# JoshuaQSH/FALCON-TTDforGNNs

Measured on NVIDIA B200. Metric: TT-EmbeddingBag rows/s fwd+bwd+SGD, higher is better.
Workload: dtype f32

## Files before the change

falcon-ttdforgnns_b200/csrc/common.cuh:

```cuda
#pragma once

#include <cuda_runtime.h>
#include <stdint.h>
#include <stdio.h>
#include <string.h>

#include "../../include/ttg_b200.h"

#if defined(__CUDA_ARCH__) && (__CUDA_ARCH__ < 1000)
#error "ttg_b200 is written for sm_100a (B200) only"
#endif

namespace ttg {

constexpr int kWarp = 32;
constexpr int kNumSMs = 148;

void set_error(const char* fmt, ...);
void count_launch(int n = 1);

#define TTG_CHECK_ARG(cond, ...)  \
  do {                            \
    if (!(cond)) {                \
      ttg::set_error(__VA_ARGS__); \
// ... 151 lines not shown
struct MmaPlan {
  const uint32_t* skeys;
  const int32_t* srow;
  const int32_t* cnt;
  const int32_t* base;
  float* Ttab;
  float* S;
  float* d0parts;
  uint32_t first_key;
  int32_t spare_sms;
};
bool mma_supported(const TTDev& tt);
bool mma_fwd_supported(const TTDev& tt);
int mma_table(const TTDev& tt, const MmaPlan& pl, bool tf32, bool chained, cudaStream_t stream);
int mma_forward(const TTDev& tt, int64_t nnz, uint32_t total_rows, const MmaPlan& pl, float* output,
                bool tf32, cudaStream_t stream);
int mma_backward(const TTDev& tt, int64_t nnz, uint32_t total_rows, const MmaPlan& pl,
                 const float* d_output, float* const* dcore, int32_t optim, float lr, float eps,
                 float* const* state, bool tf32, cudaStream_t stream);

int mma_cores_finalize(const TTDev& tt, const MmaPlan& pl, float* const* dcore, int32_t optim, float lr,
                       float eps, float* const* state, bool tf32, cudaStream_t stream);

struct RPlan {
  const uint32_t* skeys;
  const int32_t* srow;
  const int32_t* cnt;
  const int32_t* base;
  float* tab;
  float* S1;
  float* d0parts;
  float* d2parts;
};
bool r_supported(const TTDev& tt);
// ... 16 lines not shown
```

falcon-ttdforgnns_b200/csrc/tt_mma.cu:

```cuda
#include <stdlib.h>

#include <type_traits>

#include "common.cuh"

namespace ttg {

namespace {

constexpr int kThreads = 512;
constexpr int kWarps = kThreads / 32;
constexpr int kCoreThreads = 256;
constexpr int cores_warps(int c) { return c <= 80 ? 16 : 8; }
constexpr int kCoreWarps = kCoreThreads / 32;
constexpr uint32_t kInvalid = 0xffffffffu;
constexpr size_t kSmemMax = 227 * 1024;

template <int TERMS>
struct Frag {
  uint32_t hi, lo;
  __device__ __forceinline__ void set(float x) {
    if (TERMS == 3) {
      hi = (__float_as_uint(x) + 0x1000u) & 0xffffe000u;
      lo = __float_as_uint(x - __uint_as_float(hi));
// ... 85 lines not shown
          smem_u32(sdst)),
      "l"(gsrc), "r"(bytes), "r"(smem_u32(bar))
      : "memory");
}
__device__ __forceinline__ void mbar_wait(uint64_t* bar, uint32_t parity) {
  asm volatile(
      "{\n"
      ".reg .pred p;\n"
      "WAIT_%=:\n"
      "mbarrier.try_wait.parity.shared::cta.b64 p, [%0], %1;\n"
      "@p bra DONE_%=;\n"
      "bra WAIT_%=;\n"
      "DONE_%=:\n"
      "}\n" ::"r"(smem_u32(bar)),
      "r"(parity)
      : "memory");
}

constexpr int kStageU = 6;
template <int NT, typename F>
__device__ __forceinline__ void stage_core2(const float* __restrict__ core2, int nelem, F&& put) {
  const int n4 = nelem / 4;
  for (int base4 = 0; base4 < n4; base4 += NT * kStageU) {
    float4 v[kStageU];
#pragma unroll
    for (int u = 0; u < kStageU; ++u) {
      const int i4 = base4 + u * NT + (int)threadIdx.x;
      v[u] = (i4 < n4) ? ldg4(core2 + 4 * i4) : make_float4(0.f, 0.f, 0.f, 0.f);
    }
#pragma unroll
// ... 112 lines not shown
          b[1].set_split(bh.y, 0.f);
        }
        mma_terms<TERMS>(acc, a[ks], b);
      }
      if (d0) *reinterpret_cast<float2*>(d0 + 8 * nt) = make_float2(acc[0], acc[1]);
      if (d1) *reinterpret_cast<float2*>(d1 + 8 * nt) = make_float2(acc[2], acc[3]);
    }
  }
}

constexpr int tile_rows(int q2) { return 16 / q2; }
constexpr int fwd_rb(int q2) { return (16 / tile_rows(q2)) * tile_rows(q2); }
constexpr int bwd_rb(int q2) { return (q2 <= 5 ? 3 : 4) * tile_rows(q2); }
constexpr int kC2Stride = 20;

struct PairSlot {
  int row;
  int j2;
};
template <int Q2>
__device__ __forceinline__ PairSlot pair_slot(int p) {
  PairSlot s;
  s.row = p / Q2;
  s.j2 = p - s.row * Q2;
  if (p >= tile_rows(Q2) * Q2) {
    s.row = 99;
    s.j2 = 0;
  }
  return s;
}

template <int Q0, int Q1, int Q2, int R2, int TERMS, bool C2S>
__global__ void __launch_bounds__(kThreads, 1)
mma_fwd_kernel(TTDev tt, int64_t nnz, uint32_t total_rows, const uint32_t* __restrict__ skeys,
               const int32_t* __restrict__ srow, const float* __restrict__ Ttab,
               float* __restrict__ output, int rows_per_warp, int npairs_c2, int dbg,
               uint32_t first_key) {
  constexpr int A = Q0 * Q1;
  constexpr int D = A * Q2;
  constexpr int NTL = (A + 7) / 8;
  constexpr int KS = R2 / 8;
  constexpr int TR = tile_rows(Q2);
  constexpr int RB = fwd_rb(Q2);
  constexpr int CS = kC2Stride;
  static_assert(R2 % 8 == 0 && (!C2S || R2 == 16), "shared-memory core2 layout is written for r2 = 16");
  static_assert(D % 4 == 0 && A % 2 == 0 && 2 * RB <= 32, "layout");
  extern __shared__ __align__(128) float smem[];
  float* c2hi = smem;
  float* c2lo = smem + (size_t)npairs_c2 * CS;
  float* stage_all = smem + (C2S ? (size_t)npairs_c2 * CS * (TERMS == 3 ? 2 : 1) : 0);

  const int lane = threadIdx.x & 31, wib = threadIdx.x >> 5;
  const int gid = lane >> 2, tid = lane & 3;
  pdl_trigger();
  if (C2S) {
    stage_core2<kThreads>(tt.core[2], npairs_c2 * 16, [&](int e, float v) {
      const int i2row = e / (16 * Q2), rem = e % (16 * Q2);
      const int k2 = rem / Q2, j2 = rem % Q2;
      const int dst = (i2row * Q2 + j2) * CS + k2;
      if (TERMS == 3) {
        const float hi = tf32_hi(v);
        c2hi[dst] = hi;
        c2lo[dst] = v - hi;
      } else {
        c2hi[dst] = __uint_as_float(__float_as_uint(v) + 0x1000u);
      }
    });
    __syncthreads();
  }
  pdl_wait();

  const uint32_t p2 = tt.p[2];
  const uint32_t num_rows32 = (uint32_t)tt.num_rows;
  float* stage = stage_all + (size_t)wib * RB * D;
  const int64_t gw = (int64_t)blockIdx.x * kWarps + wib;
  const int64_t s_begin = gw * rows_per_warp;
  const int64_t s_end = (s_begin + rows_per_warp < nnz) ? s_begin + rows_per_warp : nnz;
  if (s_begin >= s_end) return;

  const PairSlot sl0 = pair_slot<Q2>(gid), sl1 = pair_slot<Q2>(gid + 8);
  const bool last_nt_ok = (8 * (NTL - 1) + 2 * tid + 1) < A;

  Frag<TERMS> bt[NTL][KS][2];
  float traw[NTL][KS][2];
  uint32_t g_held = kInvalid, g_pref = kInvalid;
  auto load_T = [&](uint32_t gq) {
    const float* tp = Ttab + (size_t)gq * (A * R2) + gid * R2 + tid;
#pragma unroll
    for (int nt = 0; nt < NTL; ++nt) {
// ... 94 lines not shown
          for (int ks = 0; ks < (C2S ? KS : 0); ++ks) {
            if (TERMS == 3) {
              const float* pl0 = ph0 + (size_t)npairs_c2 * CS;
              const float* pl1 = ph1 + (size_t)npairs_c2 * CS;
              af[ks][0].set_split(ph0[8 * ks], pl0[8 * ks]);
              af[ks][1].set_split(ph1[8 * ks], pl1[8 * ks]);
              af[ks][2].set_split(ph0[8 * ks + 4], pl0[8 * ks + 4]);
              af[ks][3].set_split(ph1[8 * ks + 4], pl1[8 * ks + 4]);
            } else {
              af[ks][0].set_split(ph0[8 * ks], 0.f);
              af[ks][1].set_split(ph1[8 * ks], 0.f);
              af[ks][2].set_split(ph0[8 * ks + 4], 0.f);
              af[ks][3].set_split(ph1[8 * ks + 4], 0.f);
            }
          }
          float* s0 = stage + r0 * D + sl0.j2 + 2 * tid * Q2;
          float* s1 = stage + r1 * D + sl1.j2 + 2 * tid * Q2;
          float acc[NTL][4];
#pragma unroll
          for (int nt = 0; nt < NTL; ++nt) acc[nt][0] = acc[nt][1] = acc[nt][2] = acc[nt][3] = 0.f;
#pragma unroll
          for (int ks = 0; ks < KS; ++ks)
#pragma unroll
            for (int term = first_term(TERMS); term < 3; ++term)
#pragma unroll
              for (int nt = 0; nt < NTL; ++nt) mma_term<TERMS>(term, acc[nt], af[ks], bt[nt][ks]);
#pragma unroll
          for (int nt = 0; nt < NTL; ++nt) {
            const bool cv = (8 * nt + 7 < A) || last_nt_ok;
            if (cv && v0) {
              s0[8 * nt * Q2] = acc[nt][0];
              s0[8 * nt * Q2 + Q2] = acc[nt][1];
            }
            if (cv && v1) {
              s1[8 * nt * Q2] = acc[nt][2];
              s1[8 * nt * Q2 + Q2] = acc[nt][3];
            }
          }
        }
      }
      fence_proxy_async();
      __syncwarp();
      if (skeys == nullptr) {
        if (lane == 0 && !(dbg & 1)) {
          bulk_store(output + (w0 + h * RB) * D, stage, (uint32_t)(nrows * D * 4));
          bulk_commit();
        }
        continue;
      }
      {
        const int src = h * RB + (lane < RB ? lane : 0);
        const uint32_t k_r = __shfl_sync(0xffffffffu, key, src);
        const int32_t sr_r = __shfl_sync(0xffffffffu, sr, src);
        if (lane < nrows && k_r < total_rows && !(dbg & 1)) {
          float* dst = output + (int64_t)(sr_r & 0x7fffffff) * D;
          if (sr_r >= 0)
            bulk_store(dst, stage + lane * D, D * 4);
          else
            bulk_reduce_add(dst, stage + lane * D, D * 4);
          bulk_commit();
        }
      }
    }
  }
  bulk_wait_read0();
}

template <int Q0, int Q1, int Q2, int R2, int TERMS>
__global__ void __launch_bounds__(kThreads, 1)
mma_bwd_rows_kernel(TTDev tt, int64_t nnz, uint32_t total_rows, int32_t num_groups,
                    const uint32_t* __restrict__ skeys, const int32_t* __restrict__ srow,
                    const int32_t* __restrict__ cnt, const int32_t* __restrict__ base,
                    const float* __restrict__ d_output, const float* __restrict__ Ttab,
                    float* __restrict__ Sbuf, float* __restrict__ dcore2, int npairs_c2,
                    int chunk_rows, int dbg) {
  constexpr int A = Q0 * Q1;
  constexpr int D = A * Q2;
  constexpr int NTL = (A + 7) / 8;
  constexpr int KSA = (A + 7) / 8;
  constexpr int A4 = A / 4;
  constexpr int TR = tile_rows(Q2);
  constexpr int RB = bwd_rb(Q2);
  static_assert(R2 == 16 && A % 4 == 0, "backward fragment layout is written for r2 = 16");
  extern __shared__ __align__(128) float smem[];
  float* c2s = smem;
  float* acc2 = smem + (size_t)npairs_c2 * 16;
  float* ring_all = acc2 + (size_t)npairs_c2 * 16;
  uint64_t* bars = reinterpret_cast<uint64_t*>(ring_all + (size_t)kWarps * 2 * RB * D);

  const int lane = threadIdx.x & 31, wib = threadIdx.x >> 5;
  const int gid = lane >> 2, tid = lane & 3;
  pdl_trigger();
  stage_core2<kThreads>(tt.core[2], npairs_c2 * 16, [&](int e, float v) {
    const int i2row = e / (16 * Q2), rem = e % (16 * Q2);
    const int k2 = rem / Q2, j2 = rem % Q2;
    const int pair = i2row * Q2 + j2;
    c2s[pair * 16 + bwd_slot(pair, k2)] = v;
  });
  for (int i = threadIdx.x * 4; i < npairs_c2 * 16 + kWarps * 2 * RB * D; i += kThreads * 4)
    *reinterpret_cast<float4*>(acc2 + i) = make_float4(0.f, 0.f, 0.f, 0.f);
  if (lane == 0) {
    mbar_init(bars + wib * 2, 1);
    mbar_init(bars + wib * 2 + 1, 1);
  }
  asm volatile("fence.mbarrier_init.release.cluster;" ::: "memory");
  fence_proxy_async();
  __syncthreads();
  pdl_wait();

  float* ring = ring_all + (size_t)wib * 2 * RB * D;
  uint64_t* bar = bars + wib * 2;
  uint32_t phase0 = 0, phase1 = 0;
  const uint32_t p2 = tt.p[2];
  const uint32_t num_rows32 = (uint32_t)tt.num_rows;
  const int64_t nvalid = ld_dep_s32(base + num_groups);
  const int64_t nchunks = (nvalid + chunk_rows - 1) / chunk_rows;
  const int64_t gw = (int64_t)blockIdx.x * kWarps + wib;
  const int64_t nw = (int64_t)gridDim.x * kWarps;

  const PairSlot sN0 = pair_slot<Q2>(gid), sN1 = pair_slot<Q2>(8 + gid);
  PairSlot sC[2][2];
#pragma unroll
  for (int h = 0; h < 2; ++h)
#pragma unroll
    for (int e = 0; e < 2; ++e) sC[h][e] = pair_slot<Q2>(8 * h + 2 * tid + e);
// ... 8 lines not shown
      s = (int64_t)ld_dep_s32(base + gp) + ld_dep_s32(cnt + gp);
    }
    {
      const uint32_t gl = ld_dep_u32(skeys + nom_end - 1) / p2;
      e_run = (int64_t)ld_dep_s32(base + gl) + ld_dep_s32(cnt + gl);
    }
    if (s >= e_run) continue;

    auto issue = [&](int64_t row0, int slot, int32_t r) {
      const int n = (int)((e_run - row0 < RB) ? (e_run - row0) : RB);
      if (n <= 0) return;
      if (dbg & 8) {
        if (lane == 0) mbar_expect_tx(bar + slot, 0u);
        return;
      }
      if (lane == 0) mbar_expect_tx(bar + slot, (uint32_t)(n * D * 4));
      __syncwarp();
      if (lane < n)
        bulk_load(ring + ((size_t)slot * RB + lane) * D, d_output + (int64_t)(r & 0x7fffffff) * D,
                  D * 4, bar + slot);
    };
    auto load_meta = [&](int64_t row0, uint32_t& k, int32_t& r) {
      k = total_rows;
      r = 0;
      if (lane < 2 * RB && row0 + lane < e_run) {
        k = ld_dep_u32(skeys + row0 + lane);
        r = ld_dep_s32(srow + row0 + lane);
      }
    };
    uint32_t nkey;
    int32_t nsr;
    load_meta(s, nkey, nsr);
    issue(s, 0, nsr);

    uint32_t g_cur = kInvalid, g_pref = kInvalid;
// ... 39 lines not shown
      }
    };
    auto spill_S = [&]() {
      flush_S();
      spilled = true;
      tiles_since_spill = 0;
#pragma unroll
      for (int nt = 0; nt < NTL; ++nt) Sacc[nt][0] = Sacc[nt][1] = Sacc[nt][2] = Sacc[nt][3] = 0.f;
    };

    int c2pair = 0;
    const float* buf = ring;

    auto tile = [&](auto full_tag, int rb, int nrem) {
      constexpr bool FULL = decltype(full_tag)::value;
      const float* tb = buf + rb * D;
      bool vC[2][2];
      int offC[2][2];
      const float* dC[2][2];
#pragma unroll
      for (int h = 0; h < 2; ++h)
#pragma unroll
        for (int e = 0; e < 2; ++e) {
          vC[h][e] = FULL ? (sC[h][e].row != 99) : (sC[h][e].row < nrem);
          const int rsel = vC[h][e] ? sC[h][e].row : 0;
          const int pair = __shfl_sync(0xffffffffu, c2pair, rb + rsel) + sC[h][e].j2;
          offC[h][e] = pair * 16 + (gid ^ ((pair & 2) << 2));
          dC[h][e] = tb + rsel * D + sC[h][e].j2 + gid * Q2;
        }
      const bool vN0 = FULL ? (sN0.row != 99) : (sN0.row < nrem);
      const bool vN1 = FULL ? (sN1.row != 99) : (sN1.row < nrem);
      const float* dN[2];
      dN[0] = tb + (vN0 ? sN0.row * D : 0) + sN0.j2 + tid * Q2;
      dN[1] = tb + (vN1 ? sN1.row * D : 0) + sN1.j2 + tid * Q2;

      Frag<TERMS> bn[2][KSA][2];
#pragma unroll
      for (int h = 0; h < 2; ++h)
#pragma unroll
        for (int mm = 0; mm < 2 * KSA; ++mm)
          bn[h][mm >> 1][mm & 1].set_fast((mm < A4) ? dN[h][mm * 4 * Q2] : 0.f);
      Frag<TERMS> af[2][4];
      Frag<TERMS> bs[2][NTL][2];
#pragma unroll
      for (int h = 0; h < 2; ++h)
#pragma unroll
        for (int e = 0; e < 2; ++e) {
          af[h][2 * e].set_fast(vC[h][e] ? c2s[offC[h][e]] : 0.f);
          af[h][2 * e + 1].set_fast(vC[h][e] ? c2s[offC[h][e] ^ 8] : 0.f);
// ... 48 lines not shown
      const uint32_t key = nkey;
      issue(w0 + RB, slot ^ 1, __shfl_sync(0xffffffffu, nsr, (lane < RB) ? lane + RB : 0));
      load_meta(w0 + RB, nkey, nsr);
      const uint32_t g = (key < total_rows) ? key / p2 : kInvalid;
      c2pair = (key < total_rows) ? (int)((key / num_rows32) * p2 + (key - g * p2)) * Q2 : 0;
      const uint32_t gprev = __shfl_up_sync(0xffffffffu, g, 1);
      const bool bnd = (lane < nrows) && (lane == 0 || g != gprev);
      uint32_t m = __ballot_sync(0xffffffffu, bnd);
      if (slot == 0) {
        mbar_wait(bar, phase0);
        phase0 ^= 1;
      } else {
        mbar_wait(bar + 1, phase1);
        phase1 ^= 1;
      }
      buf = ring + (size_t)slot * RB * D;
      while (m) {
        const int a = __ffs(m) - 1;
        m &= m - 1;
        const int b = m ? (__ffs(m) - 1) : nrows;
        const uint32_t gs = __shfl_sync(0xffffffffu, g, a);
        if (gs != g_cur) {
          flush_S();
          g_cur = gs;
          spilled = false;
          tiles_since_spill = 0;
#pragma unroll
          for (int nt = 0; nt < NTL; ++nt) Sacc[nt][0] = Sacc[nt][1] = Sacc[nt][2] = Sacc[nt][3] = 0.f;
          if (gs != g_pref) load_T(gs);
#pragma unroll
          for (int ks = 0; ks < KSA; ++ks)
// ... 301 lines not shown
  } else {
    const int64_t i = ((int64_t)(blockIdx.x - a.nb0 - a.nb2) * 256 + threadIdx.x) * 4;
    const int64_t n12 = a.e1 + (a.d2parts ? 0 : a.e2);
    if (i >= n12) return;
    const int t = (i < a.e1) ? 1 : 2;
    const int64_t o = (t == 1) ? i : i - a.e1;
    final_update4(a, t, o, *reinterpret_cast<const float4*>(a.dcore[t] + o));
  }
}

inline int dbg_knob(const char* name) {
  const char* v = getenv(name);
  return v ? atoi(v) : 0;
}

template <int Q0, int Q1, int Q2, int R1, int R2>
struct Shape {
  static constexpr int A = Q0 * Q1, D = Q0 * Q1 * Q2;
  static constexpr bool kC2S = (R2 == 16);
  static constexpr bool kHasBwd = (R1 == 16 && R2 == 16);

  static size_t fwd_smem(int npairs, int terms) {
    return sizeof(float) * ((kC2S ? (size_t)npairs * kC2Stride * (terms == 3 ? 2 : 1) : 0) +
                            (size_t)kWarps * fwd_rb(Q2) * D);
  }
  static size_t bwd_smem(int npairs) {
    return sizeof(float) * ((size_t)npairs * 32 + (size_t)kWarps * 2 * bwd_rb(Q2) * D) +
           sizeof(uint64_t) * kWarps * 2;
  }

  template <int TERMS>
  static int table(const TTDev& tt, const MmaPlan& pl, bool chained, cudaStream_t stream) {
    const int nb = tt.num_tables * tt.p[1];
    const int mtiles = (tt.p[0] * Q0 + 15) / 16;
    int split = (int)ceil_div(2 * kNumSMs, nb);
    if (split < 1) split = 1;
    int per = (int)ceil_div(mtiles, split);
    if (per < kCoreWarps) per = kCoreWarps;
    split = (int)ceil_div(mtiles, per);
    prof_begin(K_TABLE, stream);
    if (chained)
      TTG_CUDA(launch_pdl<2>(mma_table_kernel<Q0, Q1, R1, R2, TERMS>, dim3(nb, split), dim3(kCoreThreads), 0,
                          stream, tt, pl.Ttab, per));
    else
      mma_table_kernel<Q0, Q1, R1, R2, TERMS><<<dim3(nb, split), kCoreThreads, 0, stream>>>(tt, pl.Ttab, per);
    prof_end(K_TABLE, stream);
    TTG_LAUNCH_CHECK();
    return TTG_OK;
  }

  template <int TERMS>
  static int fwd(const TTDev& tt, int64_t nnz, uint32_t total_rows, const MmaPlan& pl, float* output,
                 cudaStream_t stream) {
    const int npairs = tt.num_tables * tt.p[2] * Q2;
    const size_t smem = fwd_smem(npairs, TERMS);
    auto kern = mma_fwd_kernel<Q0, Q1, Q2, R2, TERMS, kC2S>;
    TTG_ENSURE_SMEM(kern, smem);
    constexpr int RB = fwd_rb(Q2);
    int64_t grid = kNumSMs - pl.spare_sms;
    if (grid * kWarps * RB > nnz) grid = ceil_div(nnz, kWarps * RB);
    int64_t rpw = ceil_div(nnz, grid * kWarps);
    rpw = ceil_div(rpw, RB) * RB;
    prof_begin(K_FWD, stream);
    if (pl.skeys != nullptr)
      TTG_CUDA(launch_pdl(kern, dim3((unsigned)grid), dim3(kThreads), smem, stream, tt, nnz, total_rows,
                          pl.skeys, pl.srow, pl.Ttab, output, (int)rpw, npairs, dbg_knob("TTG_DBG_FWD"),
                          pl.first_key));
    else
      kern<<<(unsigned)grid, kThreads, smem, stream>>>(tt, nnz, total_rows, pl.skeys, pl.srow, pl.Ttab,
                                                       output, (int)rpw, npairs, dbg_knob("TTG_DBG_FWD"),
                                                       pl.first_key);
    prof_end(K_FWD, stream);
    TTG_LAUNCH_CHECK();
    return TTG_OK;
  }

  template <int TERMS>
  static int bwd(const TTDev& tt, int64_t nnz, uint32_t total_rows, const MmaPlan& pl,
                 const float* d_output, float* const* dcore, int32_t optim, float lr, float eps,
                 float* const* state, cudaStream_t stream) {
    if constexpr (!kHasBwd) {
      set_error("mma_backward: no tensor-core backward for ranks %d, %d", R1, R2);
      return TTG_ENOTSUP;
    } else {
      return bwd_impl<TERMS>(tt, nnz, total_rows, pl, d_output, dcore, optim, lr, eps, state, stream);
    }
  }

  template <int TERMS>
  static int bwd_impl(const TTDev& tt, int64_t nnz, uint32_t total_rows, const MmaPlan& pl,
                      const float* d_output, float* const* dcore, int32_t optim, float lr, float eps,
                      float* const* state, cudaStream_t stream) {
    const int npairs = tt.num_tables * tt.p[2] * Q2;
    const int64_t e2 = (int64_t)tt.num_tables * tt.p[2] * tt.cols[2];
    const int32_t groups = tt.num_tables * tt.p[0] * tt.p[1];
    TTG_CUDA(launch_pdl(mma_zero_kernel, dim3((unsigned)ceil_div(e2 / 4, 256)), dim3(256), 0, stream,
                        dcore[2], e2 / 4));
    count_launch();
    {
      const size_t smem = bwd_smem(npairs);
      auto kern = mma_bwd_rows_kernel<Q0, Q1, Q2, R2, TERMS>;
      TTG_ENSURE_SMEM(kern, smem);
      const int64_t sms = kNumSMs - pl.spare_sms;
      int64_t chunk = ceil_div(nnz, sms * kWarps);
      if (chunk < 32) chunk = 32;
      int64_t grid = ceil_div(ceil_div(nnz, chunk), kWarps);
      if (grid > sms) grid = sms;
      prof_begin(K_BWD_ROWS, stream);
      TTG_CUDA(launch_pdl(kern, dim3((unsigned)grid), dim3(kThreads), smem, stream, tt, nnz, total_rows,
                          groups, pl.skeys, pl.srow, pl.cnt, pl.base, d_output, pl.Ttab, pl.S, dcore[2],
                          npairs, (int)chunk, dbg_knob("TTG_DBG_BWD")));
      prof_end(K_BWD_ROWS, stream);
      TTG_LAUNCH_CHECK();
    }
    {
      int rc = cores<TERMS>(tt, pl, dcore[1], stream);
      if (rc != TTG_OK) return rc;
    }
    return finalize(tt, pl, dcore, optim, lr, eps, state, stream);
  }

  template <int TERMS>
  static int cores(const TTDev& tt, const MmaPlan& pl, float* dcore1, cudaStream_t stream) {
    constexpr int C = Q1 * R2;
    constexpr int NW = cores_warps(C);
    const int64_t e0 = (int64_t)tt.num_tables * tt.p[0] * tt.cols[0];
// ... 32 lines not shown
    a.nb0 = (int)ceil_div(e0, 4 * kFinCols);
    const int nb12 = (optim == TTG_OPTIM_DENSE) ? 0 : (int)ceil_div(e1 + e2, 1024);
    prof_begin(K_REDUCE, stream);
    TTG_CUDA(launch_pdl(mma_finalize_kernel, dim3(a.nb0 + nb12), dim3(256), 0, stream, a));
    prof_end(K_REDUCE, stream);
    TTG_LAUNCH_CHECK();
    return TTG_OK;
  }
};

struct MmaEntry {
  int q0, q1, q2, r1, r2;
  int a, d;
  bool has_bwd;
  int (*table[2])(const TTDev&, const MmaPlan&, bool, cudaStream_t);
  int (*fwd[2])(const TTDev&, int64_t, uint32_t, const MmaPlan&, float*, cudaStream_t);
  int (*bwd[2])(const TTDev&, int64_t, uint32_t, const MmaPlan&, const float*, float* const*,
                int32_t, float, float, float* const*, cudaStream_t);
  int (*cores[2])(const TTDev&, const MmaPlan&, float*, cudaStream_t);
  int (*finalize)(const TTDev&, const MmaPlan&, float* const*, int32_t, float, float, float* const*,
                  cudaStream_t);
  size_t (*fwd_smem)(int, int);
  size_t (*bwd_smem)(int);
};

#define TTG_MMA_SHAPE(Q0, Q1, Q2, R1, R2)                                                       \
  {                                                                                             \
    Q0, Q1, Q2, R1, R2, Q0 * Q1, Q0 * Q1 * Q2, Shape<Q0, Q1, Q2, R1, R2>::kHasBwd,              \
        {Shape<Q0, Q1, Q2, R1, R2>::table<3>, Shape<Q0, Q1, Q2, R1, R2>::table<1>},             \
        {Shape<Q0, Q1, Q2, R1, R2>::fwd<3>, Shape<Q0, Q1, Q2, R1, R2>::fwd<1>},                 \
        {Shape<Q0, Q1, Q2, R1, R2>::bwd<3>, Shape<Q0, Q1, Q2, R1, R2>::bwd<1>},                 \
        {Shape<Q0, Q1, Q2, R1, R2>::cores<3>, Shape<Q0, Q1, Q2, R1, R2>::cores<1>},             \
// ... 23 lines not shown
}

bool mma_fwd_supported(const TTDev& tt) { return find_mma(tt) != nullptr; }
bool mma_supported(const TTDev& tt) {
  const MmaEntry* e = find_mma(tt);
  return e != nullptr && e->has_bwd;
}

int mma_table(const TTDev& tt, const MmaPlan& pl, bool tf32, bool chained, cudaStream_t stream) {
  const MmaEntry* e = find_mma(tt);
  if (!e) return TTG_ENOTSUP;
  return e->table[tf32 ? 1 : 0](tt, pl, chained, stream);
}

int mma_forward(const TTDev& tt, int64_t nnz, uint32_t total_rows, const MmaPlan& pl, float* output,
                bool tf32, cudaStream_t stream) {
  const MmaEntry* e = find_mma(tt);
  if (!e) return TTG_ENOTSUP;
  return e->fwd[tf32 ? 1 : 0](tt, nnz, total_rows, pl, output, stream);
}

int mma_cores_finalize(const TTDev& tt, const MmaPlan& pl, float* const* dcore, int32_t optim, float lr,
                       float eps, float* const* state, bool tf32, cudaStream_t stream) {
  const MmaEntry* e = find_mma(tt);
  if (!e) return TTG_ENOTSUP;
  int rc = e->cores[tf32 ? 1 : 0](tt, pl, dcore[1], stream);
  if (rc != TTG_OK) return rc;
  return e->finalize(tt, pl, dcore, optim, lr, eps, state, stream);
}

int mma_finalize_parts(const TTDev& tt, const float* d0parts, int nparts, const float* d2parts, int n2parts,
                       float* const* dcore, int32_t optim, float lr, float eps, float* const* state,
                       cudaStream_t stream) {
  MmaFinalArgs a;
// ... 13 lines not shown
  }
  a.optim = optim;
  a.lr = lr;
  a.eps = eps;
  a.nb0 = (int)ceil_div(a.e0, 4 * kFinCols);
  a.nb2 = d2parts ? (int)ceil_div(a.e2, 4 * kFinCols) : 0;
  const int nb12 = (optim == TTG_OPTIM_DENSE) ? 0 : (int)ceil_div(a.e1 + (d2parts ? 0 : a.e2), 1024);
  prof_begin(K_REDUCE, stream);
  TTG_CUDA(launch_pdl(mma_finalize_kernel, dim3(a.nb0 + a.nb2 + nb12), dim3(256), 0, stream, a));
  prof_end(K_REDUCE, stream);
  TTG_LAUNCH_CHECK();
  return TTG_OK;
}

int mma_backward(const TTDev& tt, int64_t nnz, uint32_t total_rows, const MmaPlan& pl,
                 const float* d_output, float* const* dcore, int32_t optim, float lr, float eps,
                 float* const* state, bool tf32, cudaStream_t stream) {
  const MmaEntry* e = find_mma(tt);
  if (!e) return TTG_ENOTSUP;
  return e->bwd[tf32 ? 1 : 0](tt, nnz, total_rows, pl, d_output, dcore, optim, lr, eps, state, stream);
}

}
```

falcon-ttdforgnns_b200/csrc/tt_sorted.cu:

```cuda
#include <cub/device/device_radix_sort.cuh>

#include "common.cuh"

namespace ttg {

namespace {

constexpr int kFwdThreads = 256;
constexpr int kFwdRows = 4;
constexpr int kBwdThreads = 768;
constexpr int kBwdCtasPerSM = 1;
constexpr int kBwdGrid = kNumSMs * kBwdCtasPerSM;
constexpr int kBwdMinChunkRows = 32;
constexpr int kBwdStages = 3;
constexpr size_t kSmemAccLimit = 128 * 1024;
constexpr size_t kSmemCore2Limit = 64 * 1024;
constexpr uint32_t kInvalid = 0xffffffffu;
constexpr int kCoreSplit = 4;

inline bool use_group_table(const TTDev& tt, int64_t nnz) {
  const double groups = (double)tt.num_tables * tt.p[0] * tt.p[1];
  if (mma_fwd_supported(tt)) return groups <= (double)nnz;
  if ((tt.q[0] * tt.q[1]) % 2 != 0 || tt.r[2] > 16) return false;
  const double cost_group = 2.0 * tt.q[0] * tt.r[1] * tt.q[1] * tt.r[2];
// ... 1503 lines not shown
    if (!table_valid) {
      rc = r_table(tt, r_plan(w), eng, stream);
      if (rc != TTG_OK) return rc;
    }
    if (eng == 2) return r_forward(tt, nnz, r_plan(w), output, (flags & TTG_FLAG_TF32) != 0, stream);
    return rm_forward(tt, nnz, r_plan(w), output, (flags & TTG_FLAG_TF32) != 0, stream);
  }
  if (use_mma_fwd(tt, w, flags)) {
    if (zero_only) {
      rc = build_plan(tt, B, nnz, indices, rowidx, tableidx, w, false, output, true, stream);
      if (rc == TTG_OK && !table_valid) rc = mma_table(tt, mma_plan(w), (flags & TTG_FLAG_TF32) != 0, true, stream);
    } else {
      rc = table_then_plan(tt, B, nnz, indices, rowidx, tableidx, w, flags, output, stream);
    }
    if (rc != TTG_OK) return rc;
    return mma_forward(tt, nnz, total_rows, mma_plan(w, flags), output, (flags & TTG_FLAG_TF32) != 0, stream);
  }
  rc = build_plan(tt, B, nnz, indices, rowidx, tableidx, w, (flags & TTG_FLAG_DETERMINISTIC) != 0,
                  output, zero_only, stream);
  if (rc != TTG_OK) return rc;
  return e->fwd(tt, nnz, total_rows, w, output, stream);
}

int sorted_rows_range(const TTDev& tt, int64_t first_row, int64_t num, float* output, void* ws,
                      size_t ws_bytes, int32_t flags, cudaStream_t stream) {
  if (!find_entry(tt) || !mma_fwd_supported(tt) || tt.num_tables != 1) {
    set_error("rows_range: shape has no tensor-core kernels");
    return TTG_ENOTSUP;
  }
  if (first_row < 0 || num < 0 || first_row + num > tt.num_rows) {
    set_error("rows_range: [%lld, %lld) outside the table", (long long)first_row,
// ... 6 lines not shown
    return TTG_EINVAL;
  }
  const int64_t groups = (int64_t)tt.p[0] * tt.p[1];
  SortedWs w = carve(tt, 1, groups, (char*)ws);
  if (ws == nullptr || ws_bytes < w.total || w.Ttab == nullptr) {
    set_error("rows_range: workspace %zu < %zu bytes", ws_bytes, w.total);
    return TTG_ENOMEM;
  }
  MmaPlan pl = mma_plan(w);
  const bool tf32 = (flags & TTG_FLAG_TF32) != 0;
  int rc = mma_table(tt, pl, tf32, false, stream);
  if (rc != TTG_OK) return rc;
  pl.skeys = nullptr;
  pl.srow = nullptr;
  pl.first_key = (uint32_t)first_row;
  return mma_forward(tt, num, (uint32_t)tt.num_rows, pl, output, tf32, stream);
}

int sorted_plan(const TTDev& tt, int64_t B, int64_t nnz, const int64_t* indices, const int64_t* rowidx,
                const int64_t* tableidx, void* ws, size_t ws_bytes, int32_t flags, cudaStream_t stream) {
  if (!find_entry(tt)) {
    set_error("tt_plan: shape has no sorted kernels (nothing to prepare)");
    return TTG_ENOTSUP;
  }
  if (nnz == 0) return TTG_OK;
  int rc = check_common(tt, B, nnz, "tt_plan");
  if (rc != TTG_OK) return rc;
  SortedWs w = carve(tt, B, nnz, (char*)ws, (flags & TTG_FLAG_PLAN_SLOT1) ? 1 : 0);
  if (ws == nullptr || ws_bytes < w.total) {
    set_error("tt_plan: workspace %zu < %zu bytes", ws_bytes, w.total);
    return TTG_ENOMEM;
// ... 48 lines not shown
      if (rc != TTG_OK) return rc;
      rc = r_table(tt, r_plan(w), eng, stream);
      if (rc != TTG_OK) return rc;
    }
    if (eng == 1)
      return rm_backward(tt, nnz, r_plan(w), d_output, dcore, optim, lr, eps, state, (flags & TTG_FLAG_TF32) != 0,
                         stream);
    return r_backward(tt, nnz, r_plan(w), d_output, dcore, optim, lr, eps, state, (flags & TTG_FLAG_TF32) != 0,
                      stream);
  }
  if (use_mma(tt, w, flags)) {
    if (!plan_valid) {
      rc = table_then_plan(tt, B, nnz, indices, rowidx, tableidx, w, flags, nullptr, stream);
      if (rc != TTG_OK) return rc;
    }
    return mma_backward(tt, nnz, total_rows, mma_plan(w, flags), d_output, dcore, optim, lr, eps, state,
                        (flags & TTG_FLAG_TF32) != 0, stream);
  }
  if (!plan_valid) {
    rc = build_plan(tt, B, nnz, indices, rowidx, tableidx, w, (flags & TTG_FLAG_DETERMINISTIC) != 0,
                    nullptr, false, stream);
    if (rc != TTG_OK) return rc;
  }
  BwdOpt opt;
  opt.optim = optim;
  opt.lr = lr;
  opt.eps = eps;
  opt.state = state;
  opt.table_valid = plan_valid;
  opt.mma_cores = !(flags & TTG_FLAG_FFMA) && !w.smem_acc && mma_fwd_supported(tt) && !mma_supported(tt);
  opt.tf32 = (flags & TTG_FLAG_TF32) != 0;
  return e->bwd(tt, nnz, total_rows, w, d_output, dcore, opt, stream);
// ... 4 lines not shown
```

Measured before the change: 1.505 billion.

## Use TMA gather4/scatter4 tensor maps for row staging in tensor-core fwd/bwd

Builds a 2D tensor map over the output and d_output row arrays and replaces per-lane bulk copies with one TMA scatter4 per four rows in the forward kernel and gather4 loads in the backward kernel. Staging buffers are re-laid out into 32-float-aligned groups of four rows to meet TMA requirements. The intent is fewer issued copy instructions and less per-lane bulk overhead. It adds host-side tensor-map encoding on every call, slightly more shared memory, and padded out-of-range coordinates that rely on TMA bounds handling.

New measurement: 1.476 billion, median of 6. 0.981x the previous value.

```diff
diff --git a/falcon-ttdforgnns_b200/csrc/common.cuh b/falcon-ttdforgnns_b200/csrc/common.cuh
--- a/falcon-ttdforgnns_b200/csrc/common.cuh
+++ b/falcon-ttdforgnns_b200/csrc/common.cuh
@@ -189,10 +189,10 @@
 bool mma_fwd_supported(const TTDev& tt);
 int mma_table(const TTDev& tt, const MmaPlan& pl, bool tf32, bool chained, cudaStream_t stream);
 int mma_forward(const TTDev& tt, int64_t nnz, uint32_t total_rows, const MmaPlan& pl, float* output,
-                bool tf32, cudaStream_t stream);
+                int64_t out_rows, bool tf32, cudaStream_t stream);
 int mma_backward(const TTDev& tt, int64_t nnz, uint32_t total_rows, const MmaPlan& pl,
-                 const float* d_output, float* const* dcore, int32_t optim, float lr, float eps,
-                 float* const* state, bool tf32, cudaStream_t stream);
+                 const float* d_output, int64_t dout_rows, float* const* dcore, int32_t optim, float lr,
+                 float eps, float* const* state, bool tf32, cudaStream_t stream);
 
 int mma_cores_finalize(const TTDev& tt, const MmaPlan& pl, float* const* dcore, int32_t optim, float lr,
                        float eps, float* const* state, bool tf32, cudaStream_t stream);
diff --git a/falcon-ttdforgnns_b200/csrc/tt_mma.cu b/falcon-ttdforgnns_b200/csrc/tt_mma.cu
--- a/falcon-ttdforgnns_b200/csrc/tt_mma.cu
+++ b/falcon-ttdforgnns_b200/csrc/tt_mma.cu
@@ -1,3 +1,5 @@
+#include <cuda.h>
+#include <cudaTypedefs.h>
 #include <stdlib.h>
 
 #include <type_traits>
@@ -123,6 +125,31 @@
       "DONE_%=:\n"
       "}\n" ::"r"(smem_u32(bar)),
       "r"(parity)
+      : "memory");
+}
+
+__device__ __forceinline__ uint32_t warp_uniform(uint32_t v) { return __shfl_sync(0xffffffffu, v, 0); }
+__device__ __forceinline__ void tma_gather4(uint32_t sdst, const CUtensorMap* map, int32_t r0, int32_t r1,
+                                            int32_t r2, int32_t r3, uint32_t bar) {
+  asm volatile(
+      "cp.async.bulk.tensor.2d.shared::cta.global.tile::gather4.mbarrier::complete_tx::bytes"
+      " [%0], [%1, {%2, %3, %4, %5, %6}], [%7];" ::"r"(sdst),
+      "l"(map), "r"(0), "r"(r0), "r"(r1), "r"(r2), "r"(r3), "r"(bar)
+      : "memory");
+}
+__device__ __forceinline__ void tma_load_row(uint32_t sdst, const CUtensorMap* map, int32_t r, uint32_t bar) {
+  asm volatile(
+      "cp.async.bulk.tensor.2d.shared::cta.global.tile.mbarrier::complete_tx::bytes"
+      " [%0], [%1, {%2, %3}], [%4];" ::"r"(sdst),
+      "l"(map), "r"(0), "r"(r), "r"(bar)
+      : "memory");
+}
+__device__ __forceinline__ void tma_scatter4(const CUtensorMap* map, int32_t r0, int32_t r1, int32_t r2,
+                                             int32_t r3, uint32_t ssrc) {
+  asm volatile(
+      "cp.async.bulk.tensor.2d.global.shared::cta.tile::scatter4.bulk_group"
+      " [%0, {%1, %2, %3, %4, %5}], [%6];" ::"l"(map),
+      "r"(0), "r"(r0), "r"(r1), "r"(r2), "r"(r3), "r"(ssrc)
       : "memory");
 }
 
@@ -265,6 +292,14 @@
 constexpr int bwd_rb(int q2) { return (q2 <= 5 ? 3 : 4) * tile_rows(q2); }
 constexpr int kC2Stride = 20;
 
+constexpr int row_group(int d) { return (4 * d + 31) / 32 * 32; }
+template <int D>
+__device__ __forceinline__ int row_off(int r) { return (r >> 2) * row_group(D) + (r & 3) * D; }
+constexpr int fwd_stage_floats(int q2, int d) { return (fwd_rb(q2) + 3) / 4 * row_group(d); }
+constexpr int bwd_slot_floats(int q2, int d) {
+  return (bwd_rb(q2) / 4 * row_group(d) + bwd_rb(q2) % 4 * d + 31) / 32 * 32;
+}
+
 struct PairSlot {
   int row;
   int j2;
@@ -281,12 +316,11 @@
   return s;
 }
 
-template <int Q0, int Q1, int Q2, int R2, int TERMS, bool C2S>
+template <int Q0, int Q1, int Q2, int R2, int TERMS, bool C2S, bool MAP>
 __global__ void __launch_bounds__(kThreads, 1)
 mma_fwd_kernel(TTDev tt, int64_t nnz, uint32_t total_rows, const uint32_t* __restrict__ skeys,
                const int32_t* __restrict__ srow, const float* __restrict__ Ttab,
-               float* __restrict__ output, int rows_per_warp, int npairs_c2, int dbg,
-               uint32_t first_key) {
+               float* __restrict__ output, const __grid_constant__ CUtensorMap out_map, int32_t out_rows, int rows_per_warp, int npairs_c2, int dbg, uint32_t first_key) {
   constexpr int A = Q0 * Q1;
   constexpr int D = A * Q2;
   constexpr int NTL = (A + 7) / 8;
@@ -299,7 +333,7 @@
   extern __shared__ __align__(128) float smem[];
   float* c2hi = smem;
   float* c2lo = smem + (size_t)npairs_c2 * CS;
-  float* stage_all = smem + (C2S ? (size_t)npairs_c2 * CS * (TERMS == 3 ? 2 : 1) : 0);
+  float* stage_all = smem + (C2S ? ((size_t)npairs_c2 * CS * (TERMS == 3 ? 2 : 1) + 31) / 32 * 32 : 0);
 
   const int lane = threadIdx.x & 31, wib = threadIdx.x >> 5;
   const int gid = lane >> 2, tid = lane & 3;
@@ -323,7 +357,7 @@
 
   const uint32_t p2 = tt.p[2];
   const uint32_t num_rows32 = (uint32_t)tt.num_rows;
-  float* stage = stage_all + (size_t)wib * RB * D;
+  float* stage = stage_all + (size_t)wib * fwd_stage_floats(Q2, D);
   const int64_t gw = (int64_t)blockIdx.x * kWarps + wib;
   const int64_t s_begin = gw * rows_per_warp;
   const int64_t s_end = (s_begin + rows_per_warp < nnz) ? s_begin + rows_per_warp : nnz;
@@ -448,8 +482,8 @@
               af[ks][3].set_split(ph1[8 * ks + 4], 0.f);
             }
           }
-          float* s0 = stage + r0 * D + sl0.j2 + 2 * tid * Q2;
-          float* s1 = stage + r1 * D + sl1.j2 + 2 * tid * Q2;
+          float* s0 = stage + row_off<D>(r0) + sl0.j2 + 2 * tid * Q2;
+          float* s1 = stage + row_off<D>(r1) + sl1.j2 + 2 * tid * Q2;
           float acc[NTL][4];
 #pragma unroll
           for (int nt = 0; nt < NTL; ++nt) acc[nt][0] = acc[nt][1] = acc[nt][2] = acc[nt][3] = 0.f;
@@ -475,39 +509,51 @@
       }
       fence_proxy_async();
       __syncwarp();
-      if (skeys == nullptr) {
-        if (lane == 0 && !(dbg & 1)) {
-          bulk_store(output + (w0 + h * RB) * D, stage, (uint32_t)(nrows * D * 4));
+      if (dbg & 1) continue;
+      const int src = h * RB + (lane < RB ? lane : 0);
+      const uint32_t k_r = __shfl_sync(0xffffffffu, key, src);
+      const int32_t sr_r = __shfl_sync(0xffffffffu, sr, src);
+      const bool live = lane < nrows && k_r < total_rows;
+      const int64_t orow = skeys ? (int64_t)(sr_r & 0x7fffffff) : w0 + h * RB + lane;
+      if constexpr (MAP) {
+        const bool add = live && skeys != nullptr && sr_r < 0;
+        if (add) {
+          bulk_reduce_add(output + orow * D, stage + row_off<D>(lane), D * 4);
           bulk_commit();
         }
-        continue;
-      }
-      {
-        const int src = h * RB + (lane < RB ? lane : 0);
-        const uint32_t k_r = __shfl_sync(0xffffffffu, key, src);
-        const int32_t sr_r = __shfl_sync(0xffffffffu, sr, src);
-        if (lane < nrows && k_r < total_rows && !(dbg & 1)) {
-          float* dst = output + (int64_t)(sr_r & 0x7fffffff) * D;
-          if (sr_r >= 0)
-            bulk_store(dst, stage + lane * D, D * 4);
-          else
-            bulk_reduce_add(dst, stage + lane * D, D * 4);
-          bulk_commit();
+        const int32_t crd = (live && !add) ? (int32_t)orow : out_rows;
+        const uint32_t sstage = warp_uniform(smem_u32(stage));
+#pragma unroll
+        for (int q = 0; q < (RB + 3) / 4; ++q) {
+          const int32_t c0 = __shfl_sync(0xffffffffu, crd, 4 * q);
+          const int32_t c1 = __shfl_sync(0xffffffffu, crd, 4 * q + 1);
+          const int32_t c2 = __shfl_sync(0xffffffffu, crd, 4 * q + 2);
+          const int32_t c3 = __shfl_sync(0xffffffffu, crd, 4 * q + 3);
+          if (lane == 0 && !(c0 == out_rows && c1 == out_rows && c2 == out_rows && c3 == out_rows))
+            tma_scatter4(&out_map, c0, c1, c2, c3, sstage + 4 * q * row_group(D));
         }
+        if (lane == 0) bulk_commit();
+      } else if (live) {
+        float* dst = output + orow * D;
+        if (skeys != nullptr && sr_r < 0)
+          bulk_reduce_add(dst, stage + row_off<D>(lane), D * 4);
+        else
+          bulk_store(dst, stage + row_off<D>(lane), D * 4);
+        bulk_commit();
       }
     }
   }
   bulk_wait_read0();
 }
 
-template <int Q0, int Q1, int Q2, int R2, int TERMS>
+template <int Q0, int Q1, int Q2, int R2, int TERMS, bool MAP>
 __global__ void __launch_bounds__(kThreads, 1)
 mma_bwd_rows_kernel(TTDev tt, int64_t nnz, uint32_t total_rows, int32_t num_groups,
                     const uint32_t* __restrict__ skeys, const int32_t* __restrict__ srow,
                     const int32_t* __restrict__ cnt, const int32_t* __restrict__ base,
-                    const float* __restrict__ d_output, const float* __restrict__ Ttab,
-                    float* __restrict__ Sbuf, float* __restrict__ dcore2, int npairs_c2,
-                    int chunk_rows, int dbg) {
+                    const float* __restrict__ d_output, const __grid_constant__ CUtensorMap dout_map,
+                    int32_t dout_rows, const float* __restrict__ Ttab, float* __restrict__ Sbuf,
+                    float* __restrict__ dcore2, int npairs_c2, int chunk_rows, int dbg) {
   constexpr int A = Q0 * Q1;
   constexpr int D = A * Q2;
   constexpr int NTL = (A + 7) / 8;
@@ -515,12 +561,14 @@
   constexpr int A4 = A / 4;
   constexpr int TR = tile_rows(Q2);
   constexpr int RB = bwd_rb(Q2);
+  constexpr int SLOT = bwd_slot_floats(Q2, D);
   static_assert(R2 == 16 && A % 4 == 0, "backward fragment layout is written for r2 = 16");
+  static_assert(RB % 4 <= 1, "a buffer is whole gather4 groups and at most one more row");
   extern __shared__ __align__(128) float smem[];
   float* c2s = smem;
   float* acc2 = smem + (size_t)npairs_c2 * 16;
   float* ring_all = acc2 + (size_t)npairs_c2 * 16;
-  uint64_t* bars = reinterpret_cast<uint64_t*>(ring_all + (size_t)kWarps * 2 * RB * D);
+  uint64_t* bars = reinterpret_cast<uint64_t*>(ring_all + (size_t)kWarps * 2 * SLOT);
 
   const int lane = threadIdx.x & 31, wib = threadIdx.x >> 5;
   const int gid = lane >> 2, tid = lane & 3;
@@ -531,7 +579,8 @@
     const int pair = i2row * Q2 + j2;
     c2s[pair * 16 + bwd_slot(pair, k2)] = v;
   });
-  for (int i = threadIdx.x * 4; i < npairs_c2 * 16 + kWarps * 2 * RB * D; i += kThreads * 4)
+  const int nzero = npairs_c2 * 16 + (MAP ? 0 : kWarps * 2 * SLOT);
+  for (int i = threadIdx.x * 4; i < nzero; i += kThreads * 4)
     *reinterpret_cast<float4*>(acc2 + i) = make_float4(0.f, 0.f, 0.f, 0.f);
   if (lane == 0) {
     mbar_init(bars + wib * 2, 1);
@@ -542,7 +591,7 @@
   __syncthreads();
   pdl_wait();
 
-  float* ring = ring_all + (size_t)wib * 2 * RB * D;
+  float* ring = ring_all + (size_t)wib * 2 * SLOT;
   uint64_t* bar = bars + wib * 2;
   uint32_t phase0 = 0, phase1 = 0;
   const uint32_t p2 = tt.p[2];
@@ -581,11 +630,29 @@
         if (lane == 0) mbar_expect_tx(bar + slot, 0u);
         return;
       }
-      if (lane == 0) mbar_expect_tx(bar + slot, (uint32_t)(n * D * 4));
-      __syncwarp();
-      if (lane < n)
-        bulk_load(ring + ((size_t)slot * RB + lane) * D, d_output + (int64_t)(r & 0x7fffffff) * D,
-                  D * 4, bar + slot);
+      float* dst = ring + (size_t)slot * SLOT;
+      if constexpr (MAP) {
+        const int32_t crd = (lane < n) ? (r & 0x7fffffff) : dout_rows;
+        const uint32_t sdst = warp_uniform(smem_u32(dst)), sbar = warp_uniform(smem_u32(bar + slot));
+        if (lane == 0) mbar_expect_tx(bar + slot, (uint32_t)(RB * D * 4));
+#pragma unroll
+        for (int q = 0; q < RB / 4; ++q) {
+          const int32_t c0 = __shfl_sync(0xffffffffu, crd, 4 * q);
+          const int32_t c1 = __shfl_sync(0xffffffffu, crd, 4 * q + 1);
+          const int32_t c2 = __shfl_sync(0xffffffffu, crd, 4 * q + 2);
+          const int32_t c3 = __shfl_sync(0xffffffffu, crd, 4 * q + 3);
+          if (lane == 0) tma_gather4(sdst + 4 * q * row_group(D), &dout_map, c0, c1, c2, c3, sbar);
+        }
+        if (RB % 4 == 1) {
+          const int32_t c = __shfl_sync(0xffffffffu, crd, RB - 1);
+          if (lane == 0) tma_load_row(sdst + 4 * row_off<D>(RB - 1), &dout_map, c, sbar);
+        }
+      } else {
+        if (lane == 0) mbar_expect_tx(bar + slot, (uint32_t)(n * D * 4));
+        __syncwarp();
+        if (lane < n)
+          bulk_load(dst + row_off<D>(lane), d_output + (int64_t)(r & 0x7fffffff) * D, D * 4, bar + slot);
+      }
     };
     auto load_meta = [&](int64_t row0, uint32_t& k, int32_t& r) {
       k = total_rows;
@@ -655,7 +722,6 @@
 
     auto tile = [&](auto full_tag, int rb, int nrem) {
       constexpr bool FULL = decltype(full_tag)::value;
-      const float* tb = buf + rb * D;
       bool vC[2][2];
       int offC[2][2];
       const float* dC[2][2];
@@ -667,13 +733,13 @@
           const int rsel = vC[h][e] ? sC[h][e].row : 0;
           const int pair = __shfl_sync(0xffffffffu, c2pair, rb + rsel) + sC[h][e].j2;
           offC[h][e] = pair * 16 + (gid ^ ((pair & 2) << 2));
-          dC[h][e] = tb + rsel * D + sC[h][e].j2 + gid * Q2;
+          dC[h][e] = buf + row_off<D>(rb + rsel) + sC[h][e].j2 + gid * Q2;
         }
       const bool vN0 = FULL ? (sN0.row != 99) : (sN0.row < nrem);
       const bool vN1 = FULL ? (sN1.row != 99) : (sN1.row < nrem);
       const float* dN[2];
-      dN[0] = tb + (vN0 ? sN0.row * D : 0) + sN0.j2 + tid * Q2;
-      dN[1] = tb + (vN1 ? sN1.row * D : 0) + sN1.j2 + tid * Q2;
+      dN[0] = buf + row_off<D>(rb + (vN0 ? sN0.row : 0)) + sN0.j2 + tid * Q2;
+      dN[1] = buf + row_off<D>(rb + (vN1 ? sN1.row : 0)) + sN1.j2 + tid * Q2;
 
       Frag<TERMS> bn[2][KSA][2];
 #pragma unroll
@@ -752,7 +818,7 @@
         mbar_wait(bar + 1, phase1);
         phase1 ^= 1;
       }
-      buf = ring + (size_t)slot * RB * D;
+      buf = ring + (size_t)slot * SLOT;
       while (m) {
         const int a = __ffs(m) - 1;
         m &= m - 1;
@@ -1084,6 +1150,47 @@
   return v ? atoi(v) : 0;
 }
 
+int rows_map(CUtensorMap* map, bool* ok, const float* base, int64_t rows, int D) {
+  memset(map, 0, sizeof(*map));
+  *ok = base != nullptr && ((uintptr_t)base & 15) == 0 && rows >= 1 && rows < INT32_MAX &&
+        (D * 4) % 16 == 0 && D <= 256;
+  if (!*ok) return TTG_OK;
+  static PFN_cuTensorMapEncodeTiled_v12000 encode = []() -> PFN_cuTensorMapEncodeTiled_v12000 {
+    void* fn = nullptr;
+    cudaDriverEntryPointQueryResult q;
+    if (cudaGetDriverEntryPointByVersion("cuTensorMapEncodeTiled", &fn, 12000, cudaEnableDefault, &q) !=
+            cudaSuccess ||
+        q != cudaDriverEntryPointSuccess)
+      return nullptr;
+    return reinterpret_cast<PFN_cuTensorMapEncodeTiled_v12000>(fn);
+  }();
+  if (encode == nullptr) {
+    set_error("rows_map: the driver has no cuTensorMapEncodeTiled");
+    return TTG_ECUDA;
+  }
+  const cuuint64_t dims[2] = {(cuuint64_t)D, (cuuint64_t)rows};
+  const cuuint64_t pitch[1] = {(cuuint64_t)D * sizeof(float)};
+  const cuuint32_t box[2] = {(cuuint32_t)D, 1u};
+  const cuuint32_t estride[2] = {1u, 1u};
+  auto run = [&]() {
+    return encode(map, CU_TENSOR_MAP_DATA_TYPE_FLOAT32, 2, const_cast<float*>(base), dims, pitch, box, estride,
+                  CU_TENSOR_MAP_INTERLEAVE_NONE, CU_TENSOR_MAP_SWIZZLE_NONE, CU_TENSOR_MAP_L2_PROMOTION_NONE,
+                  CU_TENSOR_MAP_FLOAT_OOB_FILL_NONE);
+  };
+  CUresult r = run();
+  if (r == CUDA_ERROR_INVALID_CONTEXT) {
+    int dev = 0;
+    TTG_CUDA(cudaGetDevice(&dev));
+    TTG_CUDA(cudaSetDevice(dev));
+    r = run();
+  }
+  if (r != CUDA_SUCCESS) {
+    set_error("rows_map: cuTensorMapEncodeTiled([%lld][%d] fp32) -> CUresult %d", (long long)rows, D, (int)r);
+    return TTG_ECUDA;
+  }
+  return TTG_OK;
+}
+
 template <int Q0, int Q1, int Q2, int R1, int R2>
 struct Shape {
   static constexpr int A = Q0 * Q1, D = Q0 * Q1 * Q2;
@@ -1091,11 +1198,11 @@
   static constexpr bool kHasBwd = (R1 == 16 && R2 == 16);
 
   static size_t fwd_smem(int npairs, int terms) {
-    return sizeof(float) * ((kC2S ? (size_t)npairs * kC2Stride * (terms == 3 ? 2 : 1) : 0) +
-                            (size_t)kWarps * fwd_rb(Q2) * D);
+    return sizeof(float) * ((kC2S ? align_up((size_t)npairs * kC2Stride * (terms == 3 ? 2 : 1), 32) : 0) +
+                            (size_t)kWarps * fwd_stage_floats(Q2, D));
   }
   static size_t bwd_smem(int npairs) {
-    return sizeof(float) * ((size_t)npairs * 32 + (size_t)kWarps * 2 * bwd_rb(Q2) * D) +
+    return sizeof(float) * ((size_t)npairs * 32 + (size_t)kWarps * 2 * bwd_slot_floats(Q2, D)) +
            sizeof(uint64_t) * kWarps * 2;
   }
 
@@ -1121,11 +1228,22 @@
 
   template <int TERMS>
   static int fwd(const TTDev& tt, int64_t nnz, uint32_t total_rows, const MmaPlan& pl, float* output,
-                 cudaStream_t stream) {
+                 int64_t out_rows, cudaStream_t stream) {
     const int npairs = tt.num_tables * tt.p[2] * Q2;
+    CUtensorMap map;
+    bool use_map;
+    {
+      const int rc = rows_map(&map, &use_map, output, out_rows, D);
+      if (rc != TTG_OK) return rc;
+    }
     const size_t smem = fwd_smem(npairs, TERMS);
-    auto kern = mma_fwd_kernel<Q0, Q1, Q2, R2, TERMS, kC2S>;
-    TTG_ENSURE_SMEM(kern, smem);
+    auto kmap = mma_fwd_kernel<Q0, Q1, Q2, R2, TERMS, kC2S, true>;
+    auto krow = mma_fwd_kernel<Q0, Q1, Q2, R2, TERMS, kC2S, false>;
+    if (use_map)
+      TTG_ENSURE_SMEM(kmap, smem);
+    else
+      TTG_ENSURE_SMEM(krow, smem);
+    auto kern = use_map ? kmap : krow;
     constexpr int RB = fwd_rb(Q2);
     int64_t grid = kNumSMs - pl.spare_sms;
     if (grid * kWarps * RB > nnz) grid = ceil_div(nnz, kWarps * RB);
@@ -1134,12 +1252,12 @@
     prof_begin(K_FWD, stream);
     if (pl.skeys != nullptr)
       TTG_CUDA(launch_pdl(kern, dim3((unsigned)grid), dim3(kThreads), smem, stream, tt, nnz, total_rows,
-                          pl.skeys, pl.srow, pl.Ttab, output, (int)rpw, npairs, dbg_knob("TTG_DBG_FWD"),
-                          pl.first_key));
+                          pl.skeys, pl.srow, pl.Ttab, output, map, (int32_t)out_rows, (int)rpw, npairs,
+                          dbg_knob("TTG_DBG_FWD"), pl.first_key));
     else
       kern<<<(unsigned)grid, kThreads, smem, stream>>>(tt, nnz, total_rows, pl.skeys, pl.srow, pl.Ttab,
-                                                       output, (int)rpw, npairs, dbg_knob("TTG_DBG_FWD"),
-                                                       pl.first_key);
+                                                       output, map, (int32_t)out_rows, (int)rpw, npairs,
+                                                       dbg_knob("TTG_DBG_FWD"), pl.first_key);
     prof_end(K_FWD, stream);
     TTG_LAUNCH_CHECK();
     return TTG_OK;
@@ -1147,21 +1265,28 @@
 
   template <int TERMS>
   static int bwd(const TTDev& tt, int64_t nnz, uint32_t total_rows, const MmaPlan& pl,
-                 const float* d_output, float* const* dcore, int32_t optim, float lr, float eps,
-                 float* const* state, cudaStream_t stream) {
+                 const float* d_output, int64_t dout_rows, float* const* dcore, int32_t optim, float lr,
+                 float eps, float* const* state, cudaStream_t stream) {
     if constexpr (!kHasBwd) {
       set_error("mma_backward: no tensor-core backward for ranks %d, %d", R1, R2);
       return TTG_ENOTSUP;
     } else {
-      return bwd_impl<TERMS>(tt, nnz, total_rows, pl, d_output, dcore, optim, lr, eps, state, stream);
+      return bwd_impl<TERMS>(tt, nnz, total_rows, pl, d_output, dout_rows, dcore, optim, lr, eps, state,
+                             stream);
     }
   }
 
   template <int TERMS>
   static int bwd_impl(const TTDev& tt, int64_t nnz, uint32_t total_rows, const MmaPlan& pl,
-                      const float* d_output, float* const* dcore, int32_t optim, float lr, float eps,
-                      float* const* state, cudaStream_t stream) {
+                      const float* d_output, int64_t dout_rows, float* const* dcore, int32_t optim,
+                      float lr, float eps, float* const* state, cudaStream_t stream) {
     const int npairs = tt.num_tables * tt.p[2] * Q2;
+    CUtensorMap map;
+    bool use_map;
+    {
+      const int rc = rows_map(&map, &use_map, d_output, dout_rows, D);
+      if (rc != TTG_OK) return rc;
+    }
     const int64_t e2 = (int64_t)tt.num_tables * tt.p[2] * tt.cols[2];
     const int32_t groups = tt.num_tables * tt.p[0] * tt.p[1];
     TTG_CUDA(launch_pdl(mma_zero_kernel, dim3((unsigned)ceil_div(e2 / 4, 256)), dim3(256), 0, stream,
@@ -1169,8 +1294,13 @@
     count_launch();
     {
       const size_t smem = bwd_smem(npairs);
-      auto kern = mma_bwd_rows_kernel<Q0, Q1, Q2, R2, TERMS>;
-      TTG_ENSURE_SMEM(kern, smem);
+      auto kmap = mma_bwd_rows_kernel<Q0, Q1, Q2, R2, TERMS, true>;
+      auto krow = mma_bwd_rows_kernel<Q0, Q1, Q2, R2, TERMS, false>;
+      if (use_map)
+        TTG_ENSURE_SMEM(kmap, smem);
+      else
+        TTG_ENSURE_SMEM(krow, smem);
+      auto kern = use_map ? kmap : krow;
       const int64_t sms = kNumSMs - pl.spare_sms;
       int64_t chunk = ceil_div(nnz, sms * kWarps);
       if (chunk < 32) chunk = 32;
@@ -1178,8 +1308,8 @@
       if (grid > sms) grid = sms;
       prof_begin(K_BWD_ROWS, stream);
       TTG_CUDA(launch_pdl(kern, dim3((unsigned)grid), dim3(kThreads), smem, stream, tt, nnz, total_rows,
-                          groups, pl.skeys, pl.srow, pl.cnt, pl.base, d_output, pl.Ttab, pl.S, dcore[2],
-                          npairs, (int)chunk, dbg_knob("TTG_DBG_BWD")));
+                          groups, pl.skeys, pl.srow, pl.cnt, pl.base, d_output, map,
+                          (int32_t)dout_rows, pl.Ttab, pl.S, dcore[2], npairs, (int)chunk, dbg_knob("TTG_DBG_BWD")));
       prof_end(K_BWD_ROWS, stream);
       TTG_LAUNCH_CHECK();
     }
@@ -1242,8 +1372,8 @@
   int a, d;
   bool has_bwd;
   int (*table[2])(const TTDev&, const MmaPlan&, bool, cudaStream_t);
-  int (*fwd[2])(const TTDev&, int64_t, uint32_t, const MmaPlan&, float*, cudaStream_t);
-  int (*bwd[2])(const TTDev&, int64_t, uint32_t, const MmaPlan&, const float*, float* const*,
+  int (*fwd[2])(const TTDev&, int64_t, uint32_t, const MmaPlan&, float*, int64_t, cudaStream_t);
+  int (*bwd[2])(const TTDev&, int64_t, uint32_t, const MmaPlan&, const float*, int64_t, float* const*,
                 int32_t, float, float, float* const*, cudaStream_t);
   int (*cores[2])(const TTDev&, const MmaPlan&, float*, cudaStream_t);
   int (*finalize)(const TTDev&, const MmaPlan&, float* const*, int32_t, float, float, float* const*,
@@ -1297,10 +1427,10 @@
 }
 
 int mma_forward(const TTDev& tt, int64_t nnz, uint32_t total_rows, const MmaPlan& pl, float* output,
-                bool tf32, cudaStream_t stream) {
+                int64_t out_rows, bool tf32, cudaStream_t stream) {
   const MmaEntry* e = find_mma(tt);
   if (!e) return TTG_ENOTSUP;
-  return e->fwd[tf32 ? 1 : 0](tt, nnz, total_rows, pl, output, stream);
+  return e->fwd[tf32 ? 1 : 0](tt, nnz, total_rows, pl, output, out_rows, stream);
 }
 
 int mma_cores_finalize(const TTDev& tt, const MmaPlan& pl, float* const* dcore, int32_t optim, float lr,
@@ -1344,11 +1474,12 @@
 }
 
 int mma_backward(const TTDev& tt, int64_t nnz, uint32_t total_rows, const MmaPlan& pl,
-                 const float* d_output, float* const* dcore, int32_t optim, float lr, float eps,
-                 float* const* state, bool tf32, cudaStream_t stream) {
+                 const float* d_output, int64_t dout_rows, float* const* dcore, int32_t optim, float lr,
+                 float eps, float* const* state, bool tf32, cudaStream_t stream) {
   const MmaEntry* e = find_mma(tt);
   if (!e) return TTG_ENOTSUP;
-  return e->bwd[tf32 ? 1 : 0](tt, nnz, total_rows, pl, d_output, dcore, optim, lr, eps, state, stream);
-}
-
-}
+  return e->bwd[tf32 ? 1 : 0](tt, nnz, total_rows, pl, d_output, dout_rows, dcore, optim, lr, eps, state,
+                              stream);
+}
+
+}
diff --git a/falcon-ttdforgnns_b200/csrc/tt_sorted.cu b/falcon-ttdforgnns_b200/csrc/tt_sorted.cu
--- a/falcon-ttdforgnns_b200/csrc/tt_sorted.cu
+++ b/falcon-ttdforgnns_b200/csrc/tt_sorted.cu
@@ -1541,7 +1541,8 @@
       rc = table_then_plan(tt, B, nnz, indices, rowidx, tableidx, w, flags, output, stream);
     }
     if (rc != TTG_OK) return rc;
-    return mma_forward(tt, nnz, total_rows, mma_plan(w, flags), output, (flags & TTG_FLAG_TF32) != 0, stream);
+    return mma_forward(tt, nnz, total_rows, mma_plan(w, flags), output, (int64_t)tt.num_tables * B,
+                       (flags & TTG_FLAG_TF32) != 0, stream);
   }
   rc = build_plan(tt, B, nnz, indices, rowidx, tableidx, w, (flags & TTG_FLAG_DETERMINISTIC) != 0,
                   output, zero_only, stream);
@@ -1578,7 +1579,7 @@
   pl.skeys = nullptr;
   pl.srow = nullptr;
   pl.first_key = (uint32_t)first_row;
-  return mma_forward(tt, num, (uint32_t)tt.num_rows, pl, output, tf32, stream);
+  return mma_forward(tt, num, (uint32_t)tt.num_rows, pl, output, num, tf32, stream);
 }
 
 int sorted_plan(const TTDev& tt, int64_t B, int64_t nnz, const int64_t* indices, const int64_t* rowidx,
@@ -1657,8 +1658,8 @@
       rc = table_then_plan(tt, B, nnz, indices, rowidx, tableidx, w, flags, nullptr, stream);
       if (rc != TTG_OK) return rc;
     }
-    return mma_backward(tt, nnz, total_rows, mma_plan(w, flags), d_output, dcore, optim, lr, eps, state,
-                        (flags & TTG_FLAG_TF32) != 0, stream);
+    return mma_backward(tt, nnz, total_rows, mma_plan(w, flags), d_output, (int64_t)tt.num_tables * B, dcore,
+                        optim, lr, eps, state, (flags & TTG_FLAG_TF32) != 0, stream);
   }
   if (!plan_valid) {
     rc = build_plan(tt, B, nnz, indices, rowidx, tableidx, w, (flags & TTG_FLAG_DETERMINISTIC) != 0,
```
